# FreezyLemon/rav1d

Hardware: AMD Instinct MI355X
Metric: decoded Mpixels/s (4K 10-bit 4:2:0, post-entropy reconstruction DSP) (higher is better)
Workload: dtype u16; 1 GPU; 4K10 4:2:0 3840x2160 inter frame: mc (2 refs, 30% compound) + itx residual + deblock + cdef + lr; parallelism=replicas1 (one independent stream per GPU)

## Files before the change

rav1d_amd/csrc/lr.hip:

```cpp
#include "common.h"

MI_KTL_DEFINE(lr)

namespace mi {

constexpr int kLrWin = 80;
constexpr int kWX = 8;
constexpr int kLrAB = 68;
constexpr int kNY = 8;
constexpr int kNR = 64 / kNY;
constexpr int kNT = 64 * kNY;
constexpr int kWL = (70 + kNY - 1) / kNY;

__constant__ uint16_t k_sgr_params[16][2] = {
    { 140, 3236 }, { 112, 2158 }, { 93, 1618 }, { 80, 1438 }, { 70, 1295 }, { 58, 1177 },
    { 47, 1079 },  { 37, 996 },   { 30, 925 },  { 25, 863 },  { 0, 2589 },  { 0, 1618 },
    { 0, 1177 },   { 0, 925 },    { 56, 0 },    { 22, 0 },
};

__device__ __forceinline__ unsigned sgr_x_by_x(unsigned z) {
    if (z == 0) return 255;
    if (z >= 255) return 0;
    return (256 + ((z + 1) >> 1)) / (z + 1);
}

template <typename Px>
__device__ __forceinline__ int ld_px(const uint8_t *base, int64_t stride, int y, int x) {
    return reinterpret_cast<const Px *>(base + (int64_t)y * stride)[x];
}

template <int R>
__device__ void sgr_ab(const int16_t *win, int *A, int16_t *B, int sh, int tw, unsigned s, int bdm8,
                        const uint8_t *xbyx) {
    constexpr int n = (2 * R + 1) * (2 * R + 1);
    constexpr unsigned one_by_x = n == 25 ? 164 : 455;
    constexpr int NP = 34, G = kNT / NP;
    const int g = threadIdx.x / NP, cp = threadIdx.x - g * NP;
    const int x = 2 * cp - 2;
    if (g >= G || x > tw) return;
    const int nrows = sh + 2;
    const int per = R == 2 ? (((nrows + G - 1) / G) + 1) & ~1 : (nrows + G - 1) / G;
    const int y0 = -1 + g * per, y1 = min(-1 + (g + 1) * per, sh + 1);
    if (y0 >= y1) return;
    const uint32_t *col = reinterpret_cast<const uint32_t *>(win + x - 2 + kWX);
    constexpr int W2 = kLrWin / 2;
    auto hsum = [&](int yy, int &s0, int &q0, int &s1, int &q1) {
        const uint32_t *r = col + (yy + 3) * W2;
        const uint32_t w0 = r[0], w1 = r[1], w2 = r[2];
        const int v0 = w0 & 0xffff, v1 = w0 >> 16, v2 = w1 & 0xffff, v3 = w1 >> 16, v4 = w2 & 0xffff, v5 = w2 >> 16;
        if (R == 2) {
            const int m = v1 + v2 + v3 + v4, mq = v1 * v1 + v2 * v2 + v3 * v3 + v4 * v4;
            s0 = m + v0; q0 = mq + v0 * v0; s1 = m + v5; q1 = mq + v5 * v5;
        } else {
            const int m = v2 + v3, mq = v2 * v2 + v3 * v3;
            s0 = m + v1; q0 = mq + v1 * v1; s1 = m + v4; q1 = mq + v4 * v4;
        }
    };
    int rs0[2 * R + 1], rq0[2 * R + 1], rs1[2 * R + 1], rq1[2 * R + 1];
#pragma unroll
    for (int k = 0; k < 2 * R; k++) hsum(y0 - R + k, rs0[k], rq0[k], rs1[k], rq1[k]);
    const bool c0 = x >= -1, c1 = x + 1 <= tw;
    for (int y = y0; y < y1; y++) {
        hsum(y + R, rs0[2 * R], rq0[2 * R], rs1[2 * R], rq1[2 * R]);
        if (R == 1 || !((y + 1) & 1)) {
            int sum0 = 0, sq0 = 0, sum1 = 0, sq1 = 0;
#pragma unroll
            for (int k = 0; k <= 2 * R; k++) { sum0 += rs0[k]; sq0 += rq0[k]; sum1 += rs1[k]; sq1 += rq1[k]; }
            const int sums[2] = { sum0, sum1 }, sqs[2] = { sq0, sq1 };
            const bool on[2] = { c0, c1 };
#pragma unroll
            for (int e = 0; e < 2; e++) {
                const int a = (sqs[e] + ((1 << (2 * bdm8)) >> 1)) >> (2 * bdm8);
                const int b = (sums[e] + ((1 << bdm8) >> 1)) >> bdm8;
                const unsigned p = (unsigned)max((int)__umul24((unsigned)a, (unsigned)n) - (int)__umul24((unsigned)b, (unsigned)b), 0);
                const unsigned z = (p * s + (1u << 19)) >> 20;
                const unsigned xv = xbyx[min(z, 255u)];
                if (on[e]) {
                    A[(y + 1) * kLrAB + x + e + 1] = (int)((__umul24(__umul24(xv, one_by_x), (unsigned)sums[e]) + (1u << 11)) >> 12);
                    B[(y + 1) * kLrAB + x + e + 1] = (int16_t)xv;
                }
            }
        }
#pragma unroll
        for (int k = 0; k < 2 * R; k++) { rs0[k] = rs0[k + 1]; rq0[k] = rq0[k + 1]; rs1[k] = rs1[k + 1]; rq1[k] = rq1[k + 1]; }
    }
}

template <int R>
__device__ __forceinline__ void sgr_px(const int *A, const int16_t *B, int r0, int r1, int i,
                                       const int16_t *win, int w, int acc[kNR]) {
    const int *a0 = A + i + 1;
    const int16_t *b0 = B + i + 1;
    auto ld = [&](int y, int &ca, int &sa, int &cb, int &sb) {
        const int *ar = a0 + (y + 1) * kLrAB;
        const int16_t *br = b0 + (y + 1) * kLrAB;
        ca = ar[0]; sa = ar[-1] + ar[1];
        cb = br[0]; sb = br[-1] + br[1];
    };
    if (R == 1) {
        int ca0, sa0, cb0, sb0, ca1, sa1, cb1, sb1, ca2, sa2, cb2, sb2;
        ld(r0 - 1, ca0, sa0, cb0, sb0);
        ld(r0, ca1, sa1, cb1, sb1);
#pragma unroll
        for (int q = 0; q < kNR; q++) {
            ld(r0 + q + 1, ca2, sa2, cb2, sb2);
            if (r0 + q < r1) {
                const int src = win[(r0 + q + 3) * kLrWin + i + kWX];
                const int a = (cb1 + sb1 + cb0 + cb2) * 4 + (sb0 + sb2) * 3;
                const int b = (ca1 + sa1 + ca0 + ca2) * 4 + (sa0 + sa2) * 3;
                acc[q] += w * ((b - a * src + (1 << 8)) >> 9);
            }
            ca0 = ca1; sa0 = sa1; cb0 = cb1; sb0 = sb1;
            ca1 = ca2; sa1 = sa2; cb1 = cb2; sb1 = sb2;
        }
    } else {
        int cau, sau, cbu, sbu, cad, sad, cbd, sbd;
        ld(r0 - 1, cau, sau, cbu, sbu);
#pragma unroll
        for (int q = 0; q < kNR; q += 2) {
            ld(r0 + q + 1, cad, sad, cbd, sbd);
            if (r0 + q < r1) {
                const int src = win[(r0 + q + 3) * kLrWin + i + kWX];
                const int a = (cbu + cbd) * 6 + (sbu + sbd) * 5;
                const int b = (cau + cad) * 6 + (sau + sad) * 5;
                acc[q] += w * ((b - a * src + (1 << 8)) >> 9);
            }
            if (r0 + q + 1 < r1) {
                const int src = win[(r0 + q + 4) * kLrWin + i + kWX];
                const int a = cbd * 6 + sbd * 5;
                const int b = cad * 6 + sad * 5;
                acc[q + 1] += w * ((b - a * src + (1 << 7)) >> 8);
            }
            cau = cad; sau = sad; cbu = cbd; sbu = sbd;
        }
    }
}

__device__ __forceinline__ void wiener_hor(const int16_t *win, int16_t *hor, int wr, int tw, const int (&fh)[7],
                                           int bd, int rbh, int clip_h) {
    const int cp = threadIdx.x & 31, rg = threadIdx.x >> 5, x = 2 * cp;
    if (x >= tw) return;
    for (int rr = rg; rr < wr; rr += kNT / 32) {
        const uint32_t *w = reinterpret_cast<const uint32_t *>(win + rr * kLrWin + x + kWX - 4);
        int v[10];
#pragma unroll
        for (int k = 0; k < 5; k++) {
            const uint32_t q = w[k];
            v[2 * k] = (int)(int16_t)(q & 0xffffu);
            v[2 * k + 1] = (int)(int16_t)(q >> 16);
        }
        int s0 = 1 << (bd + 6), s1 = s0;
#pragma unroll
        for (int t = 0; t < 7; t++) { s0 += v[t + 1] * fh[t]; s1 += v[t + 2] * fh[t]; }
        const int h0 = min(max((s0 + (1 << (rbh - 1))) >> rbh, 0), clip_h);
        const int h1 = min(max((s1 + (1 << (rbh - 1))) >> rbh, 0), clip_h);
        *reinterpret_cast<uint32_t *>(hor + rr * 64 + x) = (uint32_t)(h0 & 0xffff) | ((uint32_t)h1 << 16);
    }
}

__device__ __forceinline__ void sgr_pairs(int *A, int16_t *B, const int16_t *win, int sh, int tw, int bdm8, int s0,
                                          int s1, int w0, int w1, const uint8_t *xbyx, int bdmax) {
    const int cp = threadIdx.x & 31, rg = threadIdx.x >> 5, x = 2 * cp;
    const int r0 = rg * 4, r1 = min(r0 + 4, sh);
    int acc[2][4] = {};
    auto ld = [&](int y, int (&ca)[2], int (&sa)[2], int (&cb)[2], int (&sb)[2]) {
        const int *ar = A + (y + 1) * kLrAB + x;
        const int16_t *br = B + (y + 1) * kLrAB + x;
        const int2 a01 = *reinterpret_cast<const int2 *>(ar), a23 = *reinterpret_cast<const int2 *>(ar + 2);
        const uint32_t b01 = *reinterpret_cast<const uint32_t *>(br), b23 = *reinterpret_cast<const uint32_t *>(br + 2);
        const int bv0 = (int16_t)(b01 & 0xffff), bv1 = (int16_t)(b01 >> 16), bv2 = (int16_t)(b23 & 0xffff),
                  bv3 = (int16_t)(b23 >> 16);
        ca[0] = a01.y; sa[0] = a01.x + a23.x; ca[1] = a23.x; sa[1] = a01.y + a23.y;
        cb[0] = bv1; sb[0] = bv0 + bv2; cb[1] = bv2; sb[1] = bv1 + bv3;
    };
    auto src2 = [&](int j, int (&v)[2]) {
        const uint32_t q = *reinterpret_cast<const uint32_t *>(win + (j + 3) * kLrWin + x + kWX);
        v[0] = (int16_t)(q & 0xffff); v[1] = (int16_t)(q >> 16);
    };
    const bool act = x < tw && r0 < r1;
    if (s0) {
        sgr_ab<2>(win, A, B, sh, tw, (unsigned)s0, bdm8, xbyx);
        __syncthreads();
        KTL(2);
        if (act) {
            int cau[2], sau[2], cbu[2], sbu[2], cad[2], sad[2], cbd[2], sbd[2];
            ld(r0 - 1, cau, sau, cbu, sbu);
#pragma unroll
            for (int q = 0; q < 4; q += 2) {
                ld(r0 + q + 1, cad, sad, cbd, sbd);
                int v[2];
                if (r0 + q < r1) {
                    src2(r0 + q, v);
#pragma unroll
                    for (int e = 0; e < 2; e++) {
                        const int a = (cbu[e] + cbd[e]) * 6 + (sbu[e] + sbd[e]) * 5;
                        const int b = (cau[e] + cad[e]) * 6 + (sau[e] + sad[e]) * 5;
                        acc[e][q] += __mul24(w0, (b - __mul24(a, v[e]) + (1 << 8)) >> 9);
                    }
                }
                if (r0 + q + 1 < r1) {
                    src2(r0 + q + 1, v);
#pragma unroll
                    for (int e = 0; e < 2; e++) {
                        const int a = cbd[e] * 6 + sbd[e] * 5;
                        const int b = cad[e] * 6 + sad[e] * 5;
                        acc[e][q + 1] += __mul24(w0, (b - __mul24(a, v[e]) + (1 << 7)) >> 8);
                    }
                }
#pragma unroll
                for (int e = 0; e < 2; e++) { cau[e] = cad[e]; sau[e] = sad[e]; cbu[e] = cbd[e]; sbu[e] = sbd[e]; }
            }
        }
        __syncthreads();
        KTL(3);
    }
    if (s1) {
        sgr_ab<1>(win, A, B, sh, tw, (unsigned)s1, bdm8, xbyx);
        __syncthreads();
        KTL(4);
        if (act) {
            int c0[2], t0[2], d0[2], u0[2], c1[2], t1[2], d1[2], u1[2], c2[2], t2[2], d2[2], u2[2];
            ld(r0 - 1, c0, t0, d0, u0);
            ld(r0, c1, t1, d1, u1);
#pragma unroll
            for (int q = 0; q < 4; q++) {
                ld(r0 + q + 1, c2, t2, d2, u2);
                if (r0 + q < r1) {
                    int v[2];
                    src2(r0 + q, v);
#pragma unroll
                    for (int e = 0; e < 2; e++) {
                        const int a = (d1[e] + u1[e] + d0[e] + d2[e]) * 4 + (u0[e] + u2[e]) * 3;
                        const int b = (c1[e] + t1[e] + c0[e] + c2[e]) * 4 + (t0[e] + t2[e]) * 3;
                        acc[e][q] += __mul24(w1, (b - __mul24(a, v[e]) + (1 << 8)) >> 9);
                    }
                }
#pragma unroll
                for (int e = 0; e < 2; e++) {
                    c0[e] = c1[e]; t0[e] = t1[e]; d0[e] = d1[e]; u0[e] = u1[e];
                    c1[e] = c2[e]; t1[e] = t2[e]; d1[e] = d2[e]; u1[e] = u2[e];
                }
            }
        }
    }
    __syncthreads();
    if (act) {
#pragma unroll
        for (int q = 0; q < 4; q++) {
            if (r0 + q < r1) {
                int v[2];
                src2(r0 + q, v);
                const int o0 = min(max(v[0] + ((acc[0][q] + (1 << 10)) >> 11), 0), bdmax);
                const int o1 = min(max(v[1] + ((acc[1][q] + (1 << 10)) >> 11), 0), bdmax);
                *reinterpret_cast<uint32_t *>(B + (r0 + q) * 64 + x) = (uint32_t)(o0 & 0xffff) | ((uint32_t)o1 << 16);
            }
        }
    }
}

__device__ __forceinline__ void wiener_ver(const int16_t *hor, int16_t *B, int wr, int sh, int tw, const int (&fv)[7],
                                           int bd, int rbv, int bdmax) {
    const int cp = threadIdx.x & 31, rg = threadIdx.x >> 5, x = 2 * cp;
    const int r0 = rg * 4, r1 = min(r0 + 4, sh);
    if (x >= tw || r0 >= r1) return;
    const int off = 1 << (bd + rbv - 1);
    int h0[10], h1[10];
#pragma unroll
    for (int q = 0; q < 10; q++) {
        const uint32_t w = r0 + q < wr ? *reinterpret_cast<const uint32_t *>(hor + (r0 + q) * 64 + x) : 0u;
        h0[q] = (int)(w & 0xffffu);
        h1[q] = (int)(w >> 16);
    }
#pragma unroll
    for (int q = 0; q < 4; q++) {
        if (r0 + q < r1) {
            int s0 = -off, s1 = -off;
#pragma unroll
            for (int t = 0; t < 7; t++) { s0 += h0[q + t] * fv[t]; s1 += h1[q + t] * fv[t]; }
            const int o0 = min(max((s0 + (1 << (rbv - 1))) >> rbv, 0), bdmax);
            const int o1 = min(max((s1 + (1 << (rbv - 1))) >> rbv, 0), bdmax);
            *reinterpret_cast<uint32_t *>(B + (r0 + q) * 64 + x) = (uint32_t)(o0 & 0xffff) | ((uint32_t)o1 << 16);
        }
    }
}

__device__ __forceinline__ uint32_t pk2(int lo, int hi) { return (uint32_t)(lo & 0xffff) | ((uint32_t)hi << 16); }
template <typename Px>
__device__ __forceinline__ uint4 load8(const Px *p) {
    if constexpr (sizeof(Px) == 2) {
        return *reinterpret_cast<const uint4 *>(p);
    } else {
        const uint2 d = *reinterpret_cast<const uint2 *>(p);
        return make_uint4((d.x & 0xff) | ((d.x & 0xff00) << 8), ((d.x >> 16) & 0xff) | ((d.x >> 8) & 0xff0000),
                          (d.y & 0xff) | ((d.y & 0xff00) << 8), ((d.y >> 16) & 0xff) | ((d.y >> 8) & 0xff0000));
    }
}
template <typename Px>
__device__ __forceinline__ void store8(Px *p, const uint4 &u) {
    if constexpr (sizeof(Px) == 2) {
        *reinterpret_cast<uint4 *>(p) = u;
    } else {
        uint2 d;
        d.x = (u.x & 0xff) | ((u.x >> 8) & 0xff00) | ((u.y & 0xff) << 16) | ((u.y & 0xff0000) << 8);
        d.y = (u.z & 0xff) | ((u.z >> 8) & 0xff00) | ((u.w & 0xff) << 16) | ((u.w & 0xff0000) << 8);
        *reinterpret_cast<uint2 *>(p) = d;
    }
}
__device__ __forceinline__ size_t row_off(int y, int64_t st) { return (size_t)__umul24((unsigned)y, (unsigned)st); }
template <typename Px>
__device__ __forceinline__ void store_tile(const int16_t *t, uint8_t *O, int64_t st, int S, int sh, int x0, int tw) {
    for (int i = threadIdx.x; i < sh * 8; i += kNT) {
        const int r = i >> 3, c = 8 * (i & 7);
        if (c >= tw) continue;
        Px *dp = reinterpret_cast<Px *>(O + row_off(S + r, st)) + x0 + c;
        if (c + 8 <= tw) store8<Px>(dp, *reinterpret_cast<const uint4 *>(t + r * 64 + c));
        else for (int j = 0; j < tw - c; j++) dp[j] = (Px)t[r * 64 + c + j];
    }
}

__device__ __forceinline__ int stripe_start(int k, int ssv) { return k ? (64 * k - 8) >> ssv : 0; }

__device__ __forceinline__ void lr_wiener_tile(const int (&fh)[7], const int (&fv)[7], int16_t *win, int16_t *B,
                                               int16_t *hor, int sh, int tw, int bd) {
    const int tx = threadIdx.x & 63, ty = threadIdx.x >> 6;
    const int r0 = ty * kNR, r1 = min(r0 + kNR, sh);
    const int wr = sh + 6, bdmax = (1 << bd) - 1;
    {
        const int rbh = bd == 12 ? 5 : 3, rbv = bd == 12 ? 9 : 11;
        const int clip_h = (1 << (bd + 1 + 7 - rbh)) - 1;
        wiener_hor(win, hor, wr, tw, fh, bd, rbh, clip_h);
        __syncthreads();
        wiener_ver(hor, B, wr, sh, tw, fv, bd, rbv, bdmax);
        __syncthreads();
    }
}
__device__ __forceinline__ void lr_sgr_tile(int s0, int s1, int w0, int w1, int16_t *win, int *A, int16_t *B, int sh,
                                            int tw, int bd, uint8_t *xbyx ) {
    const int tx = threadIdx.x & 63, ty = threadIdx.x >> 6;
    const int r0 = ty * kNR, r1 = min(r0 + kNR, sh);
    const int bdmax = (1 << bd) - 1;
    if (threadIdx.x < 256) xbyx[threadIdx.x] = (uint8_t)sgr_x_by_x(threadIdx.x);
    __syncthreads();
    const int bdm8 = bd - 8;
    sgr_pairs(A, B, win, sh, tw, bdm8, s0, s1, w0, w1, xbyx, bdmax);
    __syncthreads();
}

template <typename Px>
__global__ __launch_bounds__(kNT) __attribute__((amdgpu_waves_per_eu(8))) void lr_kernel(LrArgs a) {
    __shared__ __attribute__((aligned(16))) int16_t win[70 * kLrWin];
    __shared__ __attribute__((aligned(16))) int A[66 * kLrAB];
    __shared__ __attribute__((aligned(16))) int16_t B[66 * kLrAB];
    int16_t *hor = reinterpret_cast<int16_t *>(A);

    KTL(0);
    const int tx = threadIdx.x & 63, ty = threadIdx.x >> 6;
    int blk = blockIdx.x;
    if (a.order) {
        blk = a.order[blk];
        if ((unsigned)blk >= (unsigned)a.blk_start[3]) return;
    }
    const int p = blk < a.blk_start[1] ? 0 : blk < a.blk_start[2] ? 1 : 2;
    const int lb = blk - a.blk_start[p];
    const int tiles = a.tiles_x[p];
    const int k = lb / tiles, ti = lb - k * tiles;
    const int ssv = p ? a.ss_ver : 0, ssh = p ? a.ss_hor : 0;
    const int pw = a.pw[p], ph = a.ph[p];
    const int x0 = ti * a.tw[p];
    const int tw = min(a.tw[p], pw - x0);
    const int S = stripe_start(k, ssv);
    const int E = min(stripe_start(k + 1, ssv), ph);
    const int sh = E - S;
    const uint8_t *C = a.src[p];
    const uint8_t *D = a.lpf[p];
    uint8_t *O = a.dst[p];
    const int64_t st = a.stride[p];
    const int r0 = ty * kNR, r1 = min(r0 + kNR, sh);

    int type = 0;
    const MiAv1RestorationUnit *u = nullptr;
    if (a.restore & (1 << p)) {
        const int us = 1 << a.unit_log2[p ? 1 : 0];
        const int nu = max(1, (pw + (us >> 1)) / us);
        const int uc = min(x0 / us, nu - 1);
        const int xu = uc * us;
        int ay = ((64 * k) >> ssv) & ~(us - 1);
        if (ay && ay + (us >> 1) > ph) ay -= us;
        ay <<= ssv;
        const int sbi = (ay >> 7) * a.sb128w + (xu >> (7 - ssh));
        const int ui = (((ay >> 6) & 1) << 1) + ((xu >> (6 - ssh)) & 1);
        u = &a.lr_mask[sbi].lr[p][ui];
        type = u->type;
    }
    if (type == 0) {
        for (int i = threadIdx.x; i < sh * 8; i += kNT) {
            const int r = i >> 3, x = x0 + 8 * (i & 7);
            if (x >= x0 + tw) continue;
            const Px *sp = reinterpret_cast<const Px *>(C + row_off(S + r, st)) + x;
            Px *dp = reinterpret_cast<Px *>(O + row_off(S + r, st)) + x;
            if (x + 8 <= x0 + tw) store8<Px>(dp, load8<Px>(sp));
            else for (int j = 0; j < x0 + tw - x; j++) dp[j] = sp[j];
        }
        KTLV(6, 0);
        KTL(5);
        return;
    }
    KTLV(6, type);

    const bool have_top = k > 0, have_bottom = E < ph;
    const int wr = sh + 6;
    constexpr int kNV = kLrWin / 8;
    constexpr int kSV = (70 * kNV + kNT - 1) / kNT;
    uint4 sv[kSV];
#pragma unroll
    for (int q = 0; q < kSV; q++) {
        sv[q] = make_uint4(0, 0, 0, 0);
        const int i = threadIdx.x + q * kNT;
        const int rr = i / kNV, x = x0 - 8 + 8 * (i % kNV), r = rr - 3;
        if (rr < wr) {
            int yy;
            const uint8_t *src;
            if (r >= 0 && r < sh) { src = C; yy = S + r; }
            else if (r < 0) { src = have_top ? D : C; yy = have_top ? S - 2 + (r == -1) : S; }
            else { src = have_bottom ? D : C; yy = have_bottom ? min(E + (r > sh), ph - 1) : E - 1; }
            const Px *row = reinterpret_cast<const Px *>(src + row_off(yy, st));
            if (x >= 0 && x + 8 <= pw) sv[q] = load8<Px>(row + x);
            else {
                int e[8];
#pragma unroll
                for (int j = 0; j < 8; j++) e[j] = row[min(max(x + j, 0), pw - 1)];
                sv[q] = make_uint4(pk2(e[0], e[1]), pk2(e[2], e[3]), pk2(e[4], e[5]), pk2(e[6], e[7]));
            }
        }
    }
#pragma unroll
    for (int q = 0; q < kSV; q++) {
        const int i = threadIdx.x + q * kNT;
        const int rr = i / kNV;
        if (rr < wr) *reinterpret_cast<uint4 *>(&win[rr * kLrWin + 8 * (i % kNV)]) = sv[q];
    }
    __syncthreads();
    KTL(1);

    const int bd = a.bd, bdmax = (1 << bd) - 1;
    if (type == 2) {
        int fh[7], fv[7];
        fh[0] = fh[6] = u->filter_h[0]; fh[1] = fh[5] = u->filter_h[1]; fh[2] = fh[4] = u->filter_h[2];
        fh[3] = 128 - 2 * (fh[0] + fh[1] + fh[2]);
        fv[0] = fv[6] = u->filter_v[0]; fv[1] = fv[5] = u->filter_v[1]; fv[2] = fv[4] = u->filter_v[2];
        fv[3] = 128 - 2 * (fv[0] + fv[1] + fv[2]);
        const int rbh = bd == 12 ? 5 : 3, rbv = bd == 12 ? 9 : 11;
        const int clip_h = (1 << (bd + 1 + 7 - rbh)) - 1;
        wiener_hor(win, hor, wr, tw, fh, bd, rbh, clip_h);
        __syncthreads();
        KTL(2);
        wiener_ver(hor, B, wr, sh, tw, fv, bd, rbv, bdmax);
        __syncthreads();
        KTL(3);
        store_tile<Px>(B, O, st, S, sh, x0, tw);
        KTL(5);
        return;
    }

    __shared__ uint8_t xbyx[256];
    if (threadIdx.x < 256) xbyx[threadIdx.x] = (uint8_t)sgr_x_by_x(threadIdx.x);
    __syncthreads();
    const int sidx = type - 3;
    const int s0 = k_sgr_params[sidx][0], s1 = k_sgr_params[sidx][1];
    const int w0 = u->sgr_weights[0];
    const int w1 = 128 - (u->sgr_weights[0] + u->sgr_weights[1]);
    const int bdm8 = bd - 8;
    sgr_pairs(A, B, win, sh, tw, bdm8, s0, s1, w0, w1, xbyx, bdmax);
    __syncthreads();
    store_tile<Px>(B, O, st, S, sh, x0, tw);
    KTL(5);
}

template <typename Px>
__global__ __launch_bounds__(kNT) void lr_call_kernel(LrCallArgs a) {
    __shared__ __attribute__((aligned(16))) int16_t win[70 * kLrWin];
    __shared__ __attribute__((aligned(16))) int A[66 * kLrAB];
    __shared__ __attribute__((aligned(16))) int16_t B[66 * kLrAB];
    int16_t *hor = reinterpret_cast<int16_t *>(A);
    const int x0 = blockIdx.x * 64, tw = min(64, a.w - x0), h = a.h;
    const bool hl = a.edges & 1, hr = a.edges & 2, ht = a.edges & 4, hb = a.edges & 8;
    const Px *p = reinterpret_cast<const Px *>(a.p), *lpf = reinterpret_cast<const Px *>(a.lpf);
    const Px *left = reinterpret_cast<const Px *>(a.left);
    for (int i = threadIdx.x; i < (h + 6) * kLrWin; i += kNT) {
        const int rr = i / kLrWin, c = i % kLrWin;
        int x = x0 - kWX + c;
        int v = 0;
        if (x >= -3 && x < a.w + 3) {
            if (!hr && x >= a.w) x = a.w - 1;
            if (!hl && x < 0) x = 0;
            const int j = rr - 3;
            if (rr < 3 && ht) v = lpf[(rr < 2 ? 0 : 1) * a.ps + x];
            else if (j >= h && hb) v = lpf[(j == h ? 6 : 7) * a.ps + x];
            else {
                const int jj = min(max(j, 0), h - 1);
                v = x < 0 ? left[jj * 4 + 1 + (x + 3)] : p[jj * a.ps + x];
            }
        }
        win[i] = (int16_t)v;
    }
    __syncthreads();
    if (a.tp.wiener) lr_wiener_tile(a.tp.fh, a.tp.fv, win, B, hor, h, tw, a.bd);
    else {
        __shared__ uint8_t xbyx[256];
        lr_sgr_tile(a.tp.s0, a.tp.s1, a.tp.w0, a.tp.w1, win, A, B, h, tw, a.bd, xbyx);
    }
    for (int i = threadIdx.x; i < h * 64; i += kNT) {
        const int r = i >> 6, c = i & 63;
        if (c < tw) reinterpret_cast<Px *>(a.out)[r * a.w + x0 + c] = (Px)B[r * 64 + c];
    }
}

int launch_lr_call(const LrCallArgs &a, int bpc, hipStream_t s) {
    const int n = (a.w + 63) / 64;
    if (bpc == 8) hipLaunchKernelGGL(lr_call_kernel<uint8_t>, dim3(n), dim3(kNT), 0, s, a);
    else hipLaunchKernelGGL(lr_call_kernel<uint16_t>, dim3(n), dim3(kNT), 0, s, a);
    return hipGetLastError() == hipSuccess ? 0 : -5;
}

int launch_lr(const LrArgs &a, int bpc, hipStream_t s) {
    const int n = a.blk_start[3];
    if (n <= 0) return 0;
    if (bpc == 8) hipLaunchKernelGGL(lr_kernel<uint8_t>, dim3(n), dim3(kNT), 0, s, a);
    else hipLaunchKernelGGL(lr_kernel<uint16_t>, dim3(n), dim3(kNT), 0, s, a);
    return hipGetLastError() == hipSuccess ? 0 : -5;
}

}
```

Before: 47220 Mpixels/s.

## Use packed dot2 intrinsics for Wiener and SGR box sums, precompute x_by_x table

Rewrites the Wiener horizontal and vertical filters to use packed 16-bit sdot2 instructions with pre-packed taps, processing row pairs and loading with wider vector accesses. The SGR box-sum accumulation now uses udot2 for horizontal sums and replaces the shifting register window with a running pair-sum recurrence. The x_by_x lookup table is built at compile time in constant memory and copied into shared memory alongside the window load, which removes a separate barrier and the per-thread divisions. The aim is to cut VALU instruction count and a sync in loop restoration. It adds reliance on dot2 availability and changes the wiener_ver read bounds, which are guarded by a static_assert.

```diff
diff --git a/rav1d_amd/csrc/lr.hip b/rav1d_amd/csrc/lr.hip
--- a/rav1d_amd/csrc/lr.hip
+++ b/rav1d_amd/csrc/lr.hip
@@ -18,11 +18,27 @@
     { 0, 1177 },   { 0, 925 },    { 56, 0 },    { 22, 0 },
 };
 
-__device__ __forceinline__ unsigned sgr_x_by_x(unsigned z) {
-    if (z == 0) return 255;
-    if (z >= 255) return 0;
-    return (256 + ((z + 1) >> 1)) / (z + 1);
-}
+constexpr unsigned sgr_x_by_x(unsigned z) {
+    return z == 0 ? 255u : z >= 255 ? 0u : (256 + ((z + 1) >> 1)) / (z + 1);
+}
+struct SgrXbyX {
+    uint32_t w[64];
+    constexpr SgrXbyX() : w() {
+        for (unsigned i = 0; i < 64; i++)
+            w[i] = sgr_x_by_x(4 * i) | sgr_x_by_x(4 * i + 1) << 8 | sgr_x_by_x(4 * i + 2) << 16 | sgr_x_by_x(4 * i + 3) << 24;
+    }
+};
+__constant__ SgrXbyX k_sgr_xbyx = SgrXbyX();
+
+typedef short lr_s16x2 __attribute__((ext_vector_type(2)));
+typedef unsigned short lr_u16x2 __attribute__((ext_vector_type(2)));
+__device__ __forceinline__ int lr_sd2(uint32_t a, uint32_t b, int acc) {
+    return __builtin_amdgcn_sdot2(__builtin_bit_cast(lr_s16x2, a), __builtin_bit_cast(lr_s16x2, b), acc, false);
+}
+__device__ __forceinline__ unsigned lr_ud2(uint32_t a, uint32_t b, unsigned acc) {
+    return __builtin_amdgcn_udot2(__builtin_bit_cast(lr_u16x2, a), __builtin_bit_cast(lr_u16x2, b), acc, false);
+}
+__device__ __forceinline__ uint32_t pk2(int lo, int hi) { return (uint32_t)(lo & 0xffff) | ((uint32_t)hi << 16); }
 
 template <typename Px>
 __device__ __forceinline__ int ld_px(const uint8_t *base, int64_t stride, int y, int x) {
@@ -44,45 +60,65 @@
     if (y0 >= y1) return;
     const uint32_t *col = reinterpret_cast<const uint32_t *>(win + x - 2 + kWX);
     constexpr int W2 = kLrWin / 2;
-    auto hsum = [&](int yy, int &s0, int &q0, int &s1, int &q1) {
+    constexpr uint32_t k11 = 0x00010001u;
+    struct Rs { unsigned s0, q0, s1, q1; };
+    auto hsum = [&](int yy) {
         const uint32_t *r = col + (yy + 3) * W2;
         const uint32_t w0 = r[0], w1 = r[1], w2 = r[2];
-        const int v0 = w0 & 0xffff, v1 = w0 >> 16, v2 = w1 & 0xffff, v3 = w1 >> 16, v4 = w2 & 0xffff, v5 = w2 >> 16;
+        Rs o;
         if (R == 2) {
-            const int m = v1 + v2 + v3 + v4, mq = v1 * v1 + v2 * v2 + v3 * v3 + v4 * v4;
-            s0 = m + v0; q0 = mq + v0 * v0; s1 = m + v5; q1 = mq + v5 * v5;
+            const unsigned sa = lr_ud2(w0, k11, lr_ud2(w1, k11, lr_ud2(w2, k11, 0u)));
+            const unsigned qa = lr_ud2(w0, w0, lr_ud2(w1, w1, lr_ud2(w2, w2, 0u)));
+            const unsigned v0 = w0 & 0xffffu, v5 = w2 >> 16;
+            o.s0 = sa - v5; o.q0 = qa - __umul24(v5, v5); o.s1 = sa - v0; o.q1 = qa - __umul24(v0, v0);
         } else {
-            const int m = v2 + v3, mq = v2 * v2 + v3 * v3;
-            s0 = m + v1; q0 = mq + v1 * v1; s1 = m + v4; q1 = mq + v4 * v4;
-        }
+            const unsigned m = lr_ud2(w1, k11, 0u), mq = lr_ud2(w1, w1, 0u);
+            const unsigned v1 = w0 >> 16, v4 = w2 & 0xffffu;
+            o.s0 = m + v1; o.q0 = mq + __umul24(v1, v1); o.s1 = m + v4; o.q1 = mq + __umul24(v4, v4);
+        }
+        return o;
     };
-    int rs0[2 * R + 1], rq0[2 * R + 1], rs1[2 * R + 1], rq1[2 * R + 1];
-#pragma unroll
-    for (int k = 0; k < 2 * R; k++) hsum(y0 - R + k, rs0[k], rq0[k], rs1[k], rq1[k]);
+    auto add = [](const Rs &a, const Rs &b) { return Rs{ a.s0 + b.s0, a.q0 + b.q0, a.s1 + b.s1, a.q1 + b.q1 }; };
     const bool c0 = x >= -1, c1 = x + 1 <= tw;
-    for (int y = y0; y < y1; y++) {
-        hsum(y + R, rs0[2 * R], rq0[2 * R], rs1[2 * R], rq1[2 * R]);
-        if (R == 1 || !((y + 1) & 1)) {
-            int sum0 = 0, sq0 = 0, sum1 = 0, sq1 = 0;
-#pragma unroll
-            for (int k = 0; k <= 2 * R; k++) { sum0 += rs0[k]; sq0 += rq0[k]; sum1 += rs1[k]; sq1 += rq1[k]; }
-            const int sums[2] = { sum0, sum1 }, sqs[2] = { sq0, sq1 };
-            const bool on[2] = { c0, c1 };
-#pragma unroll
-            for (int e = 0; e < 2; e++) {
-                const int a = (sqs[e] + ((1 << (2 * bdm8)) >> 1)) >> (2 * bdm8);
-                const int b = (sums[e] + ((1 << bdm8) >> 1)) >> bdm8;
-                const unsigned p = (unsigned)max((int)__umul24((unsigned)a, (unsigned)n) - (int)__umul24((unsigned)b, (unsigned)b), 0);
-                const unsigned z = (p * s + (1u << 19)) >> 20;
-                const unsigned xv = xbyx[min(z, 255u)];
-                if (on[e]) {
-                    A[(y + 1) * kLrAB + x + e + 1] = (int)((__umul24(__umul24(xv, one_by_x), (unsigned)sums[e]) + (1u << 11)) >> 12);
-                    B[(y + 1) * kLrAB + x + e + 1] = (int16_t)xv;
-                }
-            }
-        }
-#pragma unroll
-        for (int k = 0; k < 2 * R; k++) { rs0[k] = rs0[k + 1]; rq0[k] = rq0[k + 1]; rs1[k] = rs1[k + 1]; rq1[k] = rq1[k + 1]; }
+    auto emit = [&](int y, const Rs &t) {
+        const unsigned sums[2] = { t.s0, t.s1 }, sqs[2] = { t.q0, t.q1 };
+        const bool on[2] = { c0, c1 };
+#pragma unroll
+        for (int e = 0; e < 2; e++) {
+            const int a = (int)((sqs[e] + ((1u << (2 * bdm8)) >> 1)) >> (2 * bdm8));
+            const int b = (int)((sums[e] + ((1u << bdm8) >> 1)) >> bdm8);
+            const unsigned p = (unsigned)max((int)__umul24((unsigned)a, (unsigned)n) - (int)__umul24((unsigned)b, (unsigned)b), 0);
+            const unsigned z = (p * s + (1u << 19)) >> 20;
+            const unsigned xv = xbyx[min(z, 255u)];
+            if (on[e]) {
+                A[(y + 1) * kLrAB + x + e + 1] = (int)((__umul24(__umul24(xv, one_by_x), sums[e]) + (1u << 11)) >> 12);
+                B[(y + 1) * kLrAB + x + e + 1] = (int16_t)xv;
+            }
+        }
+    };
+    if (R == 2) {
+        Rs pa = add(hsum(y0 - 2), hsum(y0 - 1)), pb = add(hsum(y0), hsum(y0 + 1));
+        for (int y = y0; y < y1; y += 4) {
+            Rs t = add(pa, pb), nx = hsum(y + 2);
+            emit(y, add(t, nx));
+            if (y + 2 >= y1) break;
+            pa = add(nx, hsum(y + 3));
+            t = add(pb, pa); nx = hsum(y + 4);
+            emit(y + 2, add(t, nx));
+            if (y + 4 >= y1) break;
+            pb = add(nx, hsum(y + 5));
+        }
+    } else {
+        Rs ra = hsum(y0 - 1), rb = hsum(y0);
+        for (int y = y0; y < y1; y += 2) {
+            Rs t = add(ra, rb);
+            ra = hsum(y + 1);
+            emit(y, add(t, ra));
+            if (y + 1 >= y1) break;
+            t = add(rb, ra);
+            rb = hsum(y + 2);
+            emit(y + 1, add(t, rb));
+        }
     }
 }
 
@@ -140,21 +176,27 @@
                                            int bd, int rbh, int clip_h) {
     const int cp = threadIdx.x & 31, rg = threadIdx.x >> 5, x = 2 * cp;
     if (x >= tw) return;
-    for (int rr = rg; rr < wr; rr += kNT / 32) {
-        const uint32_t *w = reinterpret_cast<const uint32_t *>(win + rr * kLrWin + x + kWX - 4);
-        int v[10];
-#pragma unroll
-        for (int k = 0; k < 5; k++) {
-            const uint32_t q = w[k];
-            v[2 * k] = (int)(int16_t)(q & 0xffffu);
-            v[2 * k + 1] = (int)(int16_t)(q >> 16);
-        }
-        int s0 = 1 << (bd + 6), s1 = s0;
-#pragma unroll
-        for (int t = 0; t < 7; t++) { s0 += v[t + 1] * fh[t]; s1 += v[t + 2] * fh[t]; }
-        const int h0 = min(max((s0 + (1 << (rbh - 1))) >> rbh, 0), clip_h);
-        const int h1 = min(max((s1 + (1 << (rbh - 1))) >> rbh, 0), clip_h);
-        *reinterpret_cast<uint32_t *>(hor + rr * 64 + x) = (uint32_t)(h0 & 0xffff) | ((uint32_t)h1 << 16);
+    const uint32_t te[4] = { pk2(0, fh[0]), pk2(fh[1], fh[2]), pk2(fh[3], fh[4]), pk2(fh[5], fh[6]) };
+    const uint32_t to[4] = { pk2(fh[0], fh[1]), pk2(fh[2], fh[3]), pk2(fh[4], fh[5]), pk2(fh[6], 0) };
+    const int rnd = (1 << (bd + 6)) + (1 << (rbh - 1));
+    for (int rp = rg; 2 * rp < wr; rp += kNT / 32) {
+        uint32_t o[2][2];
+#pragma unroll
+        for (int h = 0; h < 2; h++) {
+            const int rr = 2 * rp + h;
+            const uint32_t *w = reinterpret_cast<const uint32_t *>(win + rr * kLrWin + x + kWX - 4);
+            uint32_t q[5];
+#pragma unroll
+            for (int k = 0; k < 5; k++) q[k] = w[k];
+            int s0 = rnd, s1 = rnd;
+#pragma unroll
+            for (int k = 0; k < 4; k++) { s0 = lr_sd2(q[k], te[k], s0); s1 = lr_sd2(q[k + 1], to[k], s1); }
+            const bool in = rr < wr;
+            o[0][h] = in ? (uint32_t)min(max(s0 >> rbh, 0), clip_h) : 0u;
+            o[1][h] = in ? (uint32_t)min(max(s1 >> rbh, 0), clip_h) : 0u;
+        }
+        *reinterpret_cast<uint2 *>(reinterpret_cast<uint32_t *>(hor) + rp * 64 + x) =
+            make_uint2(o[0][0] | (o[0][1] << 16), o[1][0] | (o[1][1] << 16));
     }
 }
 
@@ -258,33 +300,35 @@
     }
 }
 
-__device__ __forceinline__ void wiener_ver(const int16_t *hor, int16_t *B, int wr, int sh, int tw, const int (&fv)[7],
+__device__ __forceinline__ void wiener_ver(const int16_t *hor, int16_t *B, int sh, int tw, const int (&fv)[7],
                                            int bd, int rbv, int bdmax) {
     const int cp = threadIdx.x & 31, rg = threadIdx.x >> 5, x = 2 * cp;
     const int r0 = rg * 4, r1 = min(r0 + 4, sh);
     if (x >= tw || r0 >= r1) return;
-    const int off = 1 << (bd + rbv - 1);
-    int h0[10], h1[10];
-#pragma unroll
-    for (int q = 0; q < 10; q++) {
-        const uint32_t w = r0 + q < wr ? *reinterpret_cast<const uint32_t *>(hor + (r0 + q) * 64 + x) : 0u;
-        h0[q] = (int)(w & 0xffffu);
-        h1[q] = (int)(w >> 16);
-    }
+    static_assert(2 * (kNT / 32 - 1) + 4 < 35 && 35 * 64 <= 66 * kLrAB, "wiener_ver reads past hor");
+    const uint32_t te[4] = { pk2(fv[0], fv[1]), pk2(fv[2], fv[3]), pk2(fv[4], fv[5]), pk2(fv[6], 0) };
+    const uint32_t to[4] = { pk2(0, fv[0]), pk2(fv[1], fv[2]), pk2(fv[3], fv[4]), pk2(fv[5], fv[6]) };
+    const int rnd = (1 << (rbv - 1)) - (1 << (bd + rbv - 1));
+    uint2 hp[5];
+#pragma unroll
+    for (int j = 0; j < 5; j++) hp[j] = *reinterpret_cast<const uint2 *>(reinterpret_cast<const uint32_t *>(hor) + (2 * rg + j) * 64 + x);
 #pragma unroll
     for (int q = 0; q < 4; q++) {
         if (r0 + q < r1) {
-            int s0 = -off, s1 = -off;
-#pragma unroll
-            for (int t = 0; t < 7; t++) { s0 += h0[q + t] * fv[t]; s1 += h1[q + t] * fv[t]; }
-            const int o0 = min(max((s0 + (1 << (rbv - 1))) >> rbv, 0), bdmax);
-            const int o1 = min(max((s1 + (1 << (rbv - 1))) >> rbv, 0), bdmax);
+            int s0 = rnd, s1 = rnd;
+#pragma unroll
+            for (int k = 0; k < 4; k++) {
+                const uint32_t t = q & 1 ? to[k] : te[k];
+                s0 = lr_sd2(hp[(q >> 1) + k].x, t, s0);
+                s1 = lr_sd2(hp[(q >> 1) + k].y, t, s1);
+            }
+            const int o0 = min(max(s0 >> rbv, 0), bdmax);
+            const int o1 = min(max(s1 >> rbv, 0), bdmax);
             *reinterpret_cast<uint32_t *>(B + (r0 + q) * 64 + x) = (uint32_t)(o0 & 0xffff) | ((uint32_t)o1 << 16);
         }
     }
 }
 
-__device__ __forceinline__ uint32_t pk2(int lo, int hi) { return (uint32_t)(lo & 0xffff) | ((uint32_t)hi << 16); }
 template <typename Px>
 __device__ __forceinline__ uint4 load8(const Px *p) {
     if constexpr (sizeof(Px) == 2) {
@@ -330,17 +374,13 @@
         const int clip_h = (1 << (bd + 1 + 7 - rbh)) - 1;
         wiener_hor(win, hor, wr, tw, fh, bd, rbh, clip_h);
         __syncthreads();
-        wiener_ver(hor, B, wr, sh, tw, fv, bd, rbv, bdmax);
+        wiener_ver(hor, B, sh, tw, fv, bd, rbv, bdmax);
         __syncthreads();
     }
 }
 __device__ __forceinline__ void lr_sgr_tile(int s0, int s1, int w0, int w1, int16_t *win, int *A, int16_t *B, int sh,
-                                            int tw, int bd, uint8_t *xbyx ) {
-    const int tx = threadIdx.x & 63, ty = threadIdx.x >> 6;
-    const int r0 = ty * kNR, r1 = min(r0 + kNR, sh);
+                                            int tw, int bd, const uint8_t *xbyx ) {
     const int bdmax = (1 << bd) - 1;
-    if (threadIdx.x < 256) xbyx[threadIdx.x] = (uint8_t)sgr_x_by_x(threadIdx.x);
-    __syncthreads();
     const int bdm8 = bd - 8;
     sgr_pairs(A, B, win, sh, tw, bdm8, s0, s1, w0, w1, xbyx, bdmax);
     __syncthreads();
@@ -411,6 +451,10 @@
     const int wr = sh + 6;
     constexpr int kNV = kLrWin / 8;
     constexpr int kSV = (70 * kNV + kNT - 1) / kNT;
+    __shared__ __attribute__((aligned(16))) uint8_t xbyx[256];
+    const bool xb = type >= 3 && threadIdx.x < 64;
+    uint32_t xw = 0;
+    if (xb) xw = k_sgr_xbyx.w[threadIdx.x];
     uint4 sv[kSV];
 #pragma unroll
     for (int q = 0; q < kSV; q++) {
@@ -439,6 +483,7 @@
         const int rr = i / kNV;
         if (rr < wr) *reinterpret_cast<uint4 *>(&win[rr * kLrWin + 8 * (i % kNV)]) = sv[q];
     }
+    if (xb) reinterpret_cast<uint32_t *>(xbyx)[threadIdx.x] = xw;
     __syncthreads();
     KTL(1);
 
@@ -454,7 +499,7 @@
         wiener_hor(win, hor, wr, tw, fh, bd, rbh, clip_h);
         __syncthreads();
         KTL(2);
-        wiener_ver(hor, B, wr, sh, tw, fv, bd, rbv, bdmax);
+        wiener_ver(hor, B, sh, tw, fv, bd, rbv, bdmax);
         __syncthreads();
         KTL(3);
         store_tile<Px>(B, O, st, S, sh, x0, tw);
@@ -462,9 +507,6 @@
         return;
     }
 
-    __shared__ uint8_t xbyx[256];
-    if (threadIdx.x < 256) xbyx[threadIdx.x] = (uint8_t)sgr_x_by_x(threadIdx.x);
-    __syncthreads();
     const int sidx = type - 3;
     const int s0 = k_sgr_params[sidx][0], s1 = k_sgr_params[sidx][1];
     const int w0 = u->sgr_weights[0];
@@ -503,10 +545,11 @@
         }
         win[i] = (int16_t)v;
     }
+    __shared__ __attribute__((aligned(16))) uint8_t xbyx[256];
+    if (!a.tp.wiener && threadIdx.x < 64) reinterpret_cast<uint32_t *>(xbyx)[threadIdx.x] = k_sgr_xbyx.w[threadIdx.x];
     __syncthreads();
     if (a.tp.wiener) lr_wiener_tile(a.tp.fh, a.tp.fv, win, B, hor, h, tw, a.bd);
     else {
-        __shared__ uint8_t xbyx[256];
         lr_sgr_tile(a.tp.s0, a.tp.s1, a.tp.w0, a.tp.w1, win, A, B, h, tw, a.bd, xbyx);
     }
     for (int i = threadIdx.x; i < h * 64; i += kNT) {
```

Measured after the change: 48020 Mpixels/s, median of 6. 1.7% higher.
